# simonfuhrmann/mve

Measured on NVIDIA H100. Metric: mvs_depth_pixels_per_second, higher is better.
Workload: dtype f32

## Files before the change

### mve_b200/build.py

```python
from __future__ import annotations

import os
import subprocess

HERE = os.path.dirname(os.path.abspath(__file__))
ROOT = os.path.dirname(HERE)
LIB = os.path.join(HERE, "libb200mvs.so")
SOURCES = [os.path.join(HERE, "csrc", "b200mvs.cu"), os.path.join(HERE, "csrc", "depthmap.cu")]
DEPS = SOURCES + [os.path.join(HERE, "csrc", "patch_opt.cuh"), os.path.join(HERE, "csrc", "patch_thread.cuh"), os.path.join(HERE, "csrc", "patch_warp.cuh"),
               os.path.join(HERE, "csrc", "pset_device.cuh"), os.path.join(ROOT, "include", "b200mvs.h")]
NVCC_FLAGS = ["-gencode", "arch=compute_90a,code=sm_90a", "-lineinfo", "-O3", "-std=c++17",
              "-Xcompiler", "-fPIC", "-shared", "-Xptxas", "-v"]


def needs_build() -> bool:
    if not os.path.exists(LIB):
        return True
    t = os.path.getmtime(LIB)
    return any(os.path.getmtime(d) > t for d in DEPS)


def build(force: bool = False, verbose: bool = False) -> str:
    if not force and not needs_build():
        return LIB
    nvcc = os.environ.get("NVCC", "/usr/local/cuda/bin/nvcc")
    cmd = [nvcc] + NVCC_FLAGS + ["-o", LIB] + SOURCES
    res = subprocess.run(cmd, capture_output=True, text=True)
    if verbose or res.returncode != 0:
        print(res.stdout)
        print(res.stderr)
    if res.returncode != 0:
        raise RuntimeError("nvcc failed for libb200mvs.so")
    with open(os.path.join(HERE, "csrc", "ptxas_info.txt"), "w") as f:
        f.write(res.stderr)
    return LIB


if __name__ == "__main__":
    print(build(force=True, verbose=True))
```

### mve_b200/csrc/b200mvs.cu

```cuda
#include "../../include/b200mvs.h"
#include "patch_opt.cuh"
#include "patch_warp.cuh"
#include "patch_thread.cuh"
#include "pset_device.cuh"

#include <algorithm>
#include <cmath>
#include <cstdarg>
#include <cstddef>
#include <cstdio>
#include <cstring>
#include <cstdlib>
#include <functional>
#include <map>
#include <chrono>
#include <ctime>
#include <mutex>
#include <string>
#include <thread>
#include <atomic>
#include <vector>

using namespace b200mvs;

namespace {

thread_local std::string g_error;

struct HostLevel {
    int w = 0, h = 0, pitch = 0;
    float proj[9], invproj[9];
    uchar4* d_img = nullptr;
    uint4* d_quad = nullptr;
};

struct HostView {
    bool valid = false;
    bool has_image = false;
    int w = 0, h = 0;
    float flen = 0, paspect = 1, pp[2] = {0.5f, 0.5f}, rot[9], trans[3];
    float campos[3];
    float w2c[12];
    std::vector<HostLevel> lv;
    uchar4* d_base = nullptr;
    size_t bytes = 0;
    uint64_t last_use = 0;
};

size_t pyramid_bytes(const HostView& v)
{
    size_t texels = 0;
    for (const HostLevel& L : v.lv) texels += (size_t)L.pitch * L.h;
    return texels * (sizeof(uchar4) + sizeof(uint4));
}

// ... 545 lines not shown
    const int xs[4] = {max(0, x2 - 1), x2, min(iw - 1, x2 + 1), min(iw - 1, x2 + 2)};
    const float wr[4][4] = {{w3, w2, w2, w3}, {w2, w1, w1, w2}, {w2, w1, w1, w2}, {w3, w2, w2, w3}};
    float v0 = 0.f, v1 = 0.f, v2 = 0.f, ws = 0.f;
#pragma unroll
    for (int r = 0; r < 4; ++r) {
        const uchar4* row = in + (size_t)ys[r] * ipitch;
#pragma unroll
        for (int k = 0; k < 4; ++k) {
            const uchar4 t = row[xs[k]];
            v0 = __fadd_rn(v0, __fmul_rn((float)t.x, wr[r][k]));
            v1 = __fadd_rn(v1, __fmul_rn((float)t.y, wr[r][k]));
            v2 = __fadd_rn(v2, __fmul_rn((float)t.z, wr[r][k]));
            ws = __fadd_rn(ws, wr[r][k]);
        }
    }
    const float q0 = __fdiv_rn(v0, ws), q1 = __fdiv_rn(v1, ws), q2 = __fdiv_rn(v2, ws);
    uchar4 o;
    o.x = (unsigned char)(q0 > 0.f ? floorf(q0 + 0.5f) : ceilf(q0 - 0.5f));
    o.y = (unsigned char)(q1 > 0.f ? floorf(q1 + 0.5f) : ceilf(q1 - 0.5f));
    o.z = (unsigned char)(q2 > 0.f ? floorf(q2 + 0.5f) : ceilf(q2 - 0.5f));
    o.w = 255;
    out[(size_t)y * opitch + x] = o;
}

__global__ void k_make_quads(const uchar4* __restrict__ img, int w, int h, int pitch, uint4* __restrict__ quad)
{
    const int x = blockIdx.x * blockDim.x + threadIdx.x;
    const int y = blockIdx.y * blockDim.y + threadIdx.y;
    if (x >= w || y >= h) return;
    const int x1 = min(x + 1, w - 1), y1 = min(y + 1, h - 1);
    const unsigned* p = reinterpret_cast<const unsigned*>(img);
    uint4 q;
    q.x = p[(size_t)y * pitch + x]; q.y = p[(size_t)y * pitch + x1];
    q.z = p[(size_t)y1 * pitch + x]; q.w = p[(size_t)y1 * pitch + x1];
    quad[(size_t)y * pitch + x] = q;
}

__global__ void k_export_rgb(const uchar4* __restrict__ src, int w, int h, int pitch, uint8_t* __restrict__ dst)
{
    const int x = blockIdx.x * blockDim.x + threadIdx.x;
    const int y = blockIdx.y * blockDim.y + threadIdx.y;
    if (x >= w || y >= h) return;
    const uchar4 t = src[(size_t)y * pitch + x];
    uint8_t* p = dst + ((size_t)y * w + x) * 3;
    p[0] = t.x; p[1] = t.y; p[2] = t.z;
}

#ifndef OPT_MIN_BLOCKS
#define OPT_MIN_BLOCKS 1
#endif
constexpr int OPT_WARPS = OPT_TPB / 32;
using PatchT = b200mvs::PatchW;
using PatchT1 = b200mvs::PatchT;
constexpr size_t OPT_LUT_BYTES = sizeof(float) * (256 * LUT_STRIDE);
constexpr size_t OPT_SMEM_BYTES = OPT_LUT_BYTES + (size_t)OPT_TPB * sizeof(PatchT1) + PatchT1::MT_BYTES;
static_assert(OPT_SMEM_BYTES + 8 + 1024 <= 196 * 1024, "the patch kernels' shared memory must stay within the 196 KB carve-out");
__device__ __forceinline__ PatchT1& thread_patch(float* smem)
{
    return reinterpret_cast<PatchT1*>(reinterpret_cast<unsigned char*>(smem) + OPT_LUT_BYTES)[threadIdx.x];
}

__device__ __forceinline__ Entry load_entry(const Entry* p)
{
    const int4 a = __ldcg(reinterpret_cast<const int4*>(p));
    const int4 b = __ldcg(reinterpret_cast<const int4*>(p) + 1);
    Entry e;
    e.xy = a.x; e.jobdir = a.y; e.conf = __int_as_float(a.z); e.depth = __int_as_float(a.w);
    e.dzI = __int_as_float(b.x); e.dzJ = __int_as_float(b.y); e.slots = (unsigned)b.z; e.pad = b.w;
    return e;
}

__device__ __forceinline__ PatchIn patch_in(const Entry& e)
{
    PatchIn pi;
    pi.x = entry_x(e); pi.y = entry_y(e);
    pi.depth = e.depth; pi.dzI = e.dzI; pi.dzJ = e.dzJ; pi.slots = e.slots;
    return pi;
}

__device__ __forceinline__ unsigned long long global_timer_ns()
{
    unsigned long long t;
    asm volatile("mov.u64 %0, %%globaltimer;" : "=l"(t));
    return t;
}

__device__ __forceinline__ void optimise_entries(PatchT& p, const Entry* list, PatchOut* res, unsigned long long n,
                                                 unsigned long long* ticket, const JobParams* jobs, unsigned long long* counters)
{
    unsigned opts = 0u;
    for (;;) {
        unsigned long long w = 0ull;
        if (p.lane == 0) w = atomicAdd(ticket, 1ull);
        w = __shfl_sync(FULL, w, 0);
        if (w >= n) break;
        const Entry e = load_entry(&list[w]);
        p.begin(&jobs[entry_job(e)], patch_in(e));
        ++opts;
        while (!p.step()) {}
        PatchOut po;
        p.finish(po);
        if (p.lane == 0) res[w] = po;
    }
    if (p.lane == 0 && opts) {
        atomicAdd(&counters[C_SETS], (unsigned long long)p.n_sets);
        atomicAdd(&counters[C_OPTS], (unsigned long long)opts);
        p.n_sets = 0u;
    }
}

__device__ __forceinline__ void optimise_entries_t(PatchT1& p, const Entry* list, PatchOut* res, unsigned long long n,
                                                   unsigned long long* ticket, const JobParams* jobs, unsigned long long* counters)
{
    const int lane = threadIdx.x & 31;
    bool have = false;
    unsigned long long idx = 0ull;
    unsigned opts = 0u;
    for (;;) {
        if (!have) {
            const unsigned act = __activemask();
            const int leader = __ffs(act) - 1;
            unsigned long long base = 0ull;
            if (lane == leader) base = atomicAdd(ticket, (unsigned long long)__popc(act));
            base = __shfl_sync(act, base, leader);
            const unsigned long long w = base + (unsigned long long)__popc(act & ((1u << lane) - 1u));
            if (w >= n) break;
            idx = w;
            const Entry e = load_entry(&list[w]);
            p.begin(&jobs[entry_job(e)], patch_in(e));
            have = true;
            ++opts;
        }
        if (p.step()) {
            PatchOut po;
            p.finish(po);
            res[idx] = po;
            have = false;
        }
    }
    if (opts) {
        atomicAdd(&counters[C_SETS], (unsigned long long)p.n_sets);
        atomicAdd(&counters[C_OPTS], (unsigned long long)opts);
        p.n_sets = 0u;
    }
}

#ifndef OPT_THREAD_MIN
#define OPT_THREAD_MIN 8192
#endif

__global__ void __launch_bounds__(OPT_TPB, OPT_MIN_BLOCKS)
k_optimize(const Entry* __restrict__ in, PatchOut* __restrict__ out, int n, int mode,
           const DevSettings* __restrict__ st, const JobParams* __restrict__ jobs, const ViewParams* __restrict__ views,
           const float* __restrict__ g_lut, unsigned long long* counters)
{
    extern __shared__ float smem[];
    for (int i = threadIdx.x; i < 256 * LUT_STRIDE; i += blockDim.x) smem[i] = g_lut[i / LUT_STRIDE];
    __syncthreads();
    if (mode == 2 || (mode == 0 && n >= OPT_THREAD_MIN)) {
        PatchT1& p = thread_patch(smem);
        bind_thread(p, st, views, smem, (int)threadIdx.x);
        optimise_entries_t(p, in, out, (unsigned long long)n, &counters[C_TICKET], jobs, counters);
    } else {
        PatchT p;
        bind_thread(p, st, views, smem, (int)threadIdx.x);
        optimise_entries(p, in, out, (unsigned long long)n, &counters[C_TICKET], jobs, counters);
    }
}

__device__ __forceinline__ unsigned long long entry_key(const Entry& e)
{
    return ((unsigned long long)__float_as_uint(e.conf) << 8) | (unsigned long long)(7 - entry_dir(e));
}

struct FrontierParams {
    Entry* list[2];
    Entry* run;
    Entry* run2;
    unsigned* tile_cnt;
    unsigned long long* tile_off;
    long long n_tiles;
    PatchOut* res;
    unsigned char* written;
    unsigned long long cap;
    int n_seeds, n_jobs;
    const DevSettings* st;
    const JobParams* jobs;
    const ViewParams* views;
    const float* lut;
    unsigned long long* counters;
    FrontierCtl* ctl;
    unsigned* hist;
    int* thr_bin;
    HostMirror* host;
    volatile unsigned long long* host_filled;
    volatile int* host_cancel_job;
    int* job_cancel;
    long long thread_min;
    unsigned long long* job_run;
    int band_bins;
    int topk;
    int first_list;
};

__device__ __forceinline__ unsigned long long ld_relaxed_u64(const unsigned long long* p)
{
    unsigned long long v;
    asm volatile("ld.relaxed.gpu.global.u64 %0, [%1];" : "=l"(v) : "l"(p) : "memory");
    return v;
}
__device__ __forceinline__ void grid_barrier(unsigned long long* bar)
{
    __syncthreads();
    if (threadIdx.x == 0) {
        __threadfence();
// ... 217 lines not shown
        PHASE_END(PH_PICK);
        n_run = __ldcg(&ctl->nrun);
        if (lead) { ctl->nlist[p] = 0ull; ctl->need = 0ull; }
        }
        unsigned long long n_thread = 0ull;
        const Entry* run_cur = P.run;
        if (!seed_round && P.n_tiles > 0) {
            __shared__ unsigned long long s_big;
            if (threadIdx.x == 0) s_big = 0ull;
            __syncthreads();
            unsigned long long mine = 0ull;
            for (int j = threadIdx.x; j < P.n_jobs; j += blockDim.x) {
                const unsigned long long c = __ldcg(&P.job_run[j]);
                if (c >= (unsigned long long)P.thread_min) mine += c;
            }
            if (mine) atomicAdd(&s_big, mine);
            __syncthreads();
            n_thread = s_big;
        }
        if (n_thread > 0ull) {
            for (size_t i = gtid; i < n_run; i += gthreads) {
                const Entry e = load_entry(&P.run[i]);
                const int j = entry_job(e);
                if (__ldcg(&P.job_run[j]) < (unsigned long long)P.thread_min) continue;
                atomicAdd(&P.tile_cnt[tile_of(P.jobs[j], e)], 1u);
            }
            PHASE_END(PH_SORT);
            for (size_t b = gtid; b < (size_t)P.n_tiles; b += gthreads) {
                const unsigned c = __ldcg(&P.tile_cnt[b]);
                if (c) P.tile_off[b] = atomicAdd(&ctl->sort_cursor, (unsigned long long)c);
            }
            PHASE_END(PH_SORT);
            for (size_t i = gtid; i < n_run; i += gthreads) {
                const Entry e = load_entry(&P.run[i]);
                const int j = entry_job(e);
                if (__ldcg(&P.job_run[j]) < (unsigned long long)P.thread_min) {
                    P.run2[n_thread + take_slot(&ctl->small_cursor)] = e;
                    continue;
                }
                const long long bin = tile_of(P.jobs[j], e);
                const unsigned k = atomicSub(&P.tile_cnt[bin], 1u) - 1u;
                P.run2[__ldcg(&P.tile_off[bin]) + k] = e;
            }
            PHASE_END(PH_SORT);
            run_cur = P.run2;
        }
        const bool by_thread = n_thread > 0ull;
        if (by_thread) {
            PatchT1& pt = thread_patch(smem);
            bind_thread(pt, P.st, P.views, smem, (int)threadIdx.x);
            optimise_entries_t(pt, run_cur, P.res, n_thread, &ctl->ticket, P.jobs, cnt);
            __syncwarp();
        }
        if (n_run > n_thread) {
            PatchT pg;
            bind_thread(pg, P.st, P.views, smem, (int)threadIdx.x);
            optimise_entries(pg, run_cur + n_thread, P.res + n_thread, n_run - n_thread, by_thread ? &ctl->ticket2 : &ctl->ticket, P.jobs, cnt);
        }
        if (seed_round) {
            PHASE_END(PH_SEED);
            for (size_t i = gtid; i < (size_t)P.n_seeds; i += gthreads) {
                const float c = __ldcg(&P.res[i].conf);
                if (!(c > 0.f)) continue;
                atomicAdd(&cnt[C_SEED_OK], 1ull);
                const Entry e = load_entry(&run_cur[i]);
                const JobParams& J = P.jobs[entry_job(e)];
                atomicMax(&J.sel[pixel_of(J, e)], seed_key(c, i));
            }
            PHASE_END(PH_SELECT);
            for (size_t i = gtid; i < (size_t)P.n_seeds; i += gthreads) {
                const float c = __ldcg(&P.res[i].conf);
                if (!(c > 0.f)) continue;
                const Entry e = load_entry(&run_cur[i]);
                const int j = entry_job(e);
                const JobParams& J = P.jobs[j];
                const int idx = pixel_of(J, e);
                if (__ldcg(&J.sel[idx]) != seed_key(c, i)) continue;
                J.sel[idx] = 0ull;
                count_for_job(filled, j);
                const PatchOut r = load_result(&P.res[i]);
                write_pixel(J, idx, r);
                push_entry(P, 0, child_entry(e.xy, j, 4, r));
            }
            if (lead) ctl->ticket = 0ull;
            PHASE_END(PH_COMMIT);
            seed_round = false;
            p = 0;
            continue;
        }
        if (by_thread) PHASE_END(PH_OPT_THREAD); else PHASE_END(PH_OPT);
        for (size_t i = gtid; i < n_run; i += gthreads) {
            const Entry e = load_entry(&run_cur[i]);
            const PatchOut r = load_result(&P.res[i]);
            const int j = entry_job(e);
            const JobParams& J = P.jobs[j];
            const int idx = pixel_of(J, e);
            unsigned char w = 0;
            if (!(r.conf == 0.f)) {
                const float old = __ldcg(&J.conf[idx]);
                if (old <= 0.f) count_for_job(filled, j);
                if (old < r.conf) { write_pixel(J, idx, r); w = 1; }
            }
            P.written[i] = w;
            const unsigned act = __activemask(), wm = __ballot_sync(act, w);
            if (wm && lane == __ffs(act) - 1) atomicAdd(&ctl->need, 4ull * (unsigned long long)__popc(wm));
        }
        if (lead) {
// ... 436 lines not shown
{
    if (!ctx) return B200MVS_ERR_INVALID_ARG;
    std::lock_guard<std::mutex> lk(ctx->mtx);
    if (id < 0 || id >= (int)ctx->views.size() || !ctx->views[id].valid) return B200MVS_ERR_INVALID_ARG;
    return (int)ctx->views[id].lv.size();
}

int b200mvs_get_level(b200mvs_ctx* ctx, int id, int level, int* w, int* h, uint8_t* rgb)
{
    if (!ctx) return B200MVS_ERR_INVALID_ARG;
    std::lock_guard<std::mutex> lk(ctx->mtx);
    if (id < 0 || id >= (int)ctx->views.size() || !ctx->views[id].valid) return fail(B200MVS_ERR_INVALID_ARG, "invalid view");
    const HostView& v = ctx->views[id];
    if (level < 0 || level >= (int)v.lv.size()) return fail(B200MVS_ERR_INVALID_ARG, "invalid level");
    const HostLevel& L = v.lv[level];
    if (w) *w = L.w;
    if (h) *h = L.h;
    if (!rgb) return 0;
    if (ctx->device != B200MVS_DEVICE_NONE) CK(cudaSetDevice(ctx->device));
    pin_views(ctx, {id});
    int rc = load_views(ctx, {id}, nullptr);
    if (rc) return rc;
    uint8_t* d = nullptr;
    const size_t bytes = (size_t)L.w * L.h * 3;
    CK(dev_alloc(ctx, reinterpret_cast<void**>(&d), bytes));
    k_export_rgb<<<dim3((L.w + 31) / 32, (L.h + 7) / 8), dim3(32, 8), 0, ctx->stream>>>(L.d_img, L.w, L.h, L.pitch, d);
    cudaError_t e = cudaMemcpyAsync(rgb, d, bytes, cudaMemcpyDeviceToHost, ctx->stream);
    cudaStreamSynchronize(ctx->stream);
    dev_free(ctx, d, bytes);
    if (e != cudaSuccess) return fail(B200MVS_ERR_CUDA, "get_level copy: %s", cudaGetErrorString(e));
    return 0;
}

int b200mvs_global_view_selection(b200mvs_ctx* ctx, const b200mvs_settings* s, int ref, int32_t* ids_out, int cap)
{
    if (!ctx) return B200MVS_ERR_INVALID_ARG;
    std::lock_guard<std::mutex> lk(ctx->mtx);
    int rc;
    if ((rc = check_settings(s)) || (rc = check_ref_view(ctx, *s, ref))) return rc;
    if (cap > 0 && !ids_out) return fail(B200MVS_ERR_INVALID_ARG, "b200mvs_global_view_selection: ids_out is NULL");
    std::vector<int> sel;
    bool planned = false;
    {
        std::lock_guard<std::mutex> pl(ctx->plan_mtx);
        if (const HostPlan* p = find_plan(ctx, *s, ref)) { sel = p->gsel; planned = true; }
    }
    if (!planned) sel = global_view_selection(ctx, *s, ref);
    for (int i = 0; i < (int)sel.size() && i < cap; ++i) ids_out[i] = sel[i];
    return (int)sel.size();
}

int b200mvs_set_patch_mode(b200mvs_ctx* ctx, int mode, int64_t thread_min)
{
    if (!ctx || mode < 0 || mode > 2) return B200MVS_ERR_INVALID_ARG;
    std::lock_guard<std::mutex> lk(ctx->mtx);
    ctx->optimize_mode = mode;
    ctx->thread_min = thread_min;
    return 0;
}

int b200mvs_set_frontier_capacity(b200mvs_ctx* ctx, double entries_per_px, uint64_t min_entries)
{
    if (!ctx) return B200MVS_ERR_INVALID_ARG;
    std::lock_guard<std::mutex> lk(ctx->mtx);
    if (!std::isfinite(entries_per_px) || entries_per_px < 0.0 || entries_per_px > 64.0)
        return fail(B200MVS_ERR_INVALID_ARG, "frontier capacity: entries per pixel must be in [0, 64], got %g", entries_per_px);
    if (min_entries > (1ull << 40) || (entries_per_px == 0.0 && min_entries == 0))
        return fail(B200MVS_ERR_INVALID_ARG, "frontier capacity: min_entries must be at most 2^40, and at least 1 when entries per pixel is 0");
    ctx->frontier_cap.per_px = entries_per_px;
    ctx->frontier_cap.min = min_entries;
    return 0;
}

int b200mvs_frontier_info(b200mvs_ctx* ctx, uint64_t* initial_entries, uint64_t* final_entries, uint64_t* n_resumes)
{
    if (!ctx) return B200MVS_ERR_INVALID_ARG;
    std::lock_guard<std::mutex> lk(ctx->mtx);
    if (initial_entries) *initial_entries = ctx->fr_initial;
    if (final_entries) *final_entries = ctx->fr_final;
    if (n_resumes) *n_resumes = ctx->fr_resumes;
    return 0;
}

int b200mvs_plan_views(b200mvs_ctx* ctx, const b200mvs_settings* s, int n_refs, const int32_t* refs)
{
    if (!ctx) return B200MVS_ERR_INVALID_ARG;
    int rc = check_settings(s);
    if (rc) return rc;
    if (n_refs < 0 || (n_refs > 0 && !refs)) return fail(B200MVS_ERR_INVALID_ARG, "b200mvs_plan_views: bad arguments");
    std::vector<int> all(n_refs);
    for (int j = 0; j < n_refs; ++j) {
        if ((rc = check_ref_view(ctx, *s, refs[j]))) return rc;
        all[j] = j;
    }
    std::vector<HostPlan> made(n_refs);
    make_plans(ctx, *s, refs, all, made, nullptr);
    std::lock_guard<std::mutex> pl(ctx->plan_mtx);
    for (int j = 0; j < n_refs; ++j) ctx->plans[refs[j]] = std::move(made[j]);
    return 0;
}

int b200mvs_optimize_patches(b200mvs_ctx* ctx, const b200mvs_settings* s, int ref, const int32_t* gids, int ng,
                             const b200mvs_patch_in* in, int n, b200mvs_patch_out* out, b200mvs_stats* stats)
{
    if (!ctx) return B200MVS_ERR_INVALID_ARG;
    std::lock_guard<std::mutex> lk(ctx->mtx);
    int rc;
// ... 623 lines not shown
```

### mve_b200/csrc/patch_warp.cuh

```cuda
#pragma once
#include "patch_opt.cuh"

namespace b200mvs {

__device__ __forceinline__ float warp_sum(float v)
{
#pragma unroll
    for (int o = 16; o > 0; o >>= 1) v += __shfl_xor_sync(FULL, v, o);
    return v;
}
__device__ __forceinline__ double warp_sum(double v)
{
#pragma unroll
    for (int o = 16; o > 0; o >>= 1) v += __shfl_xor_sync(FULL, v, o);
    return v;
}
__device__ __forceinline__ float warp_max(float v)
{
#pragma unroll
    for (int o = 16; o > 0; o >>= 1) v = fmaxf(v, __shfl_xor_sync(FULL, v, o));
    return v;
}

__device__ __forceinline__ void warp_sum4(int lane, float& a, float& b, float& c, float& d)
// ... 133 lines not shown
            L.quad = reinterpret_cast<const uint4*>(__ldg(reinterpret_cast<const unsigned long long*>(&V->lv[l].quad)));
        }
        const bool aux = lane == NS;
        float qx, qy;
        project(w, L, aux ? cpx + crx : px, aux ? cpy + cry : py, aux ? cpz + crz : pz, qx, qy);
        const float ddx = __shfl_sync(FULL, qx, NS) - __shfl_sync(FULL, qx, CENTER);
        const float ddy = __shfl_sync(FULL, qy, NS) - __shfl_sync(FULL, qy, CENTER);
        const float dd2 = ddx * ddx + ddy * ddy;
        const float dd = dd2 * rsqrt_fast(dd2);
        const bool dok = dd > 0.f;
        const float step = rcp_fast(dd);
        const bool inb = qx > 0.f && qx < (float)(L.w - 1) && qy > 0.f && qy < (float)(L.h - 1);
        if (!__all_sync(FULL, inb || !act)) return 0u;
        if (act) {
            float gx = 0.f, gy = 0.f;
            if (dok) {
                float tx, ty;
                project(w, L, px + rx * step, py + ry * step, pz + rz * step, tx, ty);
                gx = tx - qx; gy = ty - qy;
            }
            const int left = (int)floorf(qx), top = (int)floorf(qy);
            const float fx = qx - (float)left, fy = qy - (float)top;
            const uint4 Q = __ldg(L.quad + (size_t)top * L.pitch + left);
            const float a[3] = {lut_k<0>(lut_tab, lane4, Q.x), lut_k<1>(lut_tab, lane4, Q.x), lut_k<2>(lut_tab, lane4, Q.x)};
            const float b[3] = {lut_k<0>(lut_tab, lane4, Q.y), lut_k<1>(lut_tab, lane4, Q.y), lut_k<2>(lut_tab, lane4, Q.y)};
            const float c[3] = {lut_k<0>(lut_tab, lane4, Q.z), lut_k<1>(lut_tab, lane4, Q.z), lut_k<2>(lut_tab, lane4, Q.z)};
            const float e[3] = {lut_k<0>(lut_tab, lane4, Q.w), lut_k<1>(lut_tab, lane4, Q.w), lut_k<2>(lut_tab, lane4, Q.w)};
#pragma unroll
            for (int ch = 0; ch < 3; ++ch) {
                const float x0 = (1.f - fx) * a[ch] + fx * b[ch];
                const float x3 = (1.f - fx) * c[ch] + fx * e[ch];
                n[ch] = (1.f - fy) * x0 + fy * x3;
                const float der = gx * (b[ch] - a[ch]) + gy * (c[ch] - a[ch]) + (gy * fx + gx * fy) * (a[ch] - b[ch] - c[ch] + e[ch]);
                d[ch] = dok ? der * dd : 0.f;
            }
        }
        return dok ? 3u : 1u;
    }

    __device__ __forceinline__ float ncc_of(const float (&n)[3]) const
    {
        const float inv_n = 1.f / (float)NS;
        float my0 = n[0], my1 = n[1], my2 = n[2], pad = 0.f;
        warp_sum4(lane, my0, my1, my2, pad);
        my0 *= inv_n; my1 *= inv_n; my2 *= inv_n;
        const float y0 = act ? n[0] - my0 : 0.f, y1 = act ? n[1] - my1 : 0.f, y2 = act ? n[2] - my2 : 0.f;
        float sqrDevY = y0 * y0 + y1 * y1 + y2 * y2;
        float devXY = e0 * y0 + e1 * y1 + e2 * y2;
        warp_sum2(lane, sqrDevY, devXY);
        const float p = sqrDevX * sqrDevY;
        return p > 0.f ? devXY * rsqrt_fast(p) : -1.f;
    }

    __device__ __forceinline__ void pass(bool candidates, bool cs_pending, bool want_ncc, bool want_normal, float*, PassOut& po)
    {
        float num = 0.f, den = 0.f;
        float A0 = 0.f, A1 = 0.f, A2 = 0.f, A3 = 0.f, A4 = 0.f, A5 = 0.f, B0 = 0.f, B1 = 0.f, B2 = 0.f;
        bool cs_active = cs_pending && st->use_color_scale;
        bool df_l = false;
        unsigned bits = 0u;
        const int count = candidates ? job->n_global : nsel();
        for (int k = 0; k < count; ++k) {
            int slot = k;
            if (candidates) { if (!((avail >> k) & 1u)) continue; }
            else slot = __shfl_sync(FULL, sel_l, k);
            float n[3], d[3];
            const unsigned r = sample(&views[job->gview[slot]], n, d);
            if (candidates) {
                const float v = (r & 1u) ? ncc_of(n) : -1.f;
                if (v < st->min_ncc) avail &= ~(1u << k);
                else if (lane == k) cand_ncc_l = v;
                continue;
            }
            if (r & 1u) bits |= 1u << (SH_COL + k);
            if (r & 2u) bits |= 1u << (SH_DER + k);
            if (want_ncc) {
                const float v = (r & 1u) ? ncc_of(n) : -1.f;
                if (lane == k) { df_l = fabsf(v - ncc_l) > st->min_refine_diff; ncc_l = v; }
            }
            float c0 = __shfl_sync(FULL, cs0_l, k), c1 = __shfl_sync(FULL, cs1_l, k), c2 = __shfl_sync(FULL, cs2_l, k);
            if (cs_active) {
                if (!(r & 1u)) cs_active = false;
                else {
                    float cc[3] = {c0, c1, c2};
                    float ab[3] = {(m0 - n[0] * c0) * n[0], (m1 - n[1] * c1) * n[1], (m2 - n[2] * c2) * n[2]};
                    float aa[3] = {n[0] * n[0], n[1] * n[1], n[2] * n[2]};
                    warp_sum4(lane, ab[0], ab[1], ab[2], aa[0]);
                    warp_sum2(lane, aa[1], aa[2]);
                    colour_scale_step(cc, ab, aa);
                    c0 = cc[0]; c1 = cc[1]; c2 = cc[2];
                    if (lane == k) { cs0_l = c0; cs1_l = c1; cs2_l = c2; }
                }
            }
            if ((r & 2u) && act) {
                const float g0 = c0 * d[0], g1 = c1 * d[1], g2 = c2 * d[2];
                const float r0 = m0 - c0 * n[0], r1 = m1 - c1 * n[1], r2 = m2 - c2 * n[2];
                num += g0 * r0 + g1 * r1 + g2 * r2;
                den += g0 * g0 + g1 * g1 + g2 * g2;
                if (want_normal) {
                    const float gg[3] = {g0, g1, g2};
                    const float rr[3] = {r0, r1, r2};
#pragma unroll
                    for (int ch = 0; ch < 3; ++ch) {
                        const float a0 = gg[ch];
                        const float a1 = fi * a0;
                        const float a2 = fj * a0;
                        A0 += a0 * a0; A1 += a0 * a1; A2 += a0 * a2;
                        A3 += a1 * a1; A4 += a1 * a2; A5 += a2 * a2;
                        B0 += a0 * rr[ch]; B1 += a1 * rr[ch]; B2 += a2 * rr[ch];
                    }
                }
            }
        }
        if (candidates) return;
        warp_sum2(lane, num, den);
        po.num = num; po.den = den;
        if (want_ncc) bits |= F_HAS_NCC | ((__ballot_sync(FULL, df_l) & 0xFu) << SH_DF);
        if (want_normal) bits |= F_HAS_NORMAL;
        pk = (pk & ~((0xFFu << SH_COL) | (want_ncc ? 0xFu << SH_DF : 0u) | F_HAS_NORMAL | F_HAS_NCC)) | bits;
        if (want_normal) {
            const double D0 = warp_sum((double)A0), D1 = warp_sum((double)A1), D2 = warp_sum((double)A2), D3 = warp_sum((double)A3);
            const double D4 = warp_sum((double)A4), D5 = warp_sum((double)A5);
            const double E0 = warp_sum((double)B0), E1 = warp_sum((double)B1), E2 = warp_sum((double)B2);
            const double m[9] = {D0, D1, D2, D1, D3, D4, D2, D4, D5};
            const double det = m[0] * m[4] * m[8] + m[1] * m[5] * m[6] + m[2] * m[3] * m[7]
                             - m[2] * m[4] * m[6] - m[1] * m[3] * m[8] - m[0] * m[5] * m[7];
            put(F_SINGULAR, det == 0.0);
            double inv[9];
            inv[0] = m[4] * m[8] - m[5] * m[7];
            inv[1] = m[2] * m[7] - m[1] * m[8];
            inv[2] = m[1] * m[5] - m[2] * m[4];
            inv[3] = m[5] * m[6] - m[3] * m[8];
            inv[4] = m[0] * m[8] - m[2] * m[6];
            inv[5] = m[2] * m[3] - m[0] * m[5];
            inv[6] = m[3] * m[7] - m[4] * m[6];
            inv[7] = m[1] * m[6] - m[0] * m[7];
            inv[8] = m[0] * m[4] - m[1] * m[3];
#pragma unroll
            for (int q = 0; q < 9; ++q) inv[q] /= det;
            po.nX0 = (float)(inv[0] * E0 + inv[1] * E1 + inv[2] * E2);
            po.nX1 = (float)(inv[3] * E0 + inv[4] * E1 + inv[5] * E2);
            po.nX2 = (float)(inv[6] * E0 + inv[7] * E1 + inv[8] * E2);
        }
    }

    __device__ __forceinline__ void sel_erase_mask(unsigned mask)
    {
        int src = 0, cnt = 0;
        for (int k = 0; k < MAX_LOCAL; ++k) {
            const bool kk = k < nsel() && !((mask >> k) & 1u);
            if (kk) { if (cnt == lane) src = k; ++cnt; }
        }
        const int s = __shfl_sync(FULL, sel_l, src);
        const float a = __shfl_sync(FULL, cs0_l, src), b = __shfl_sync(FULL, cs1_l, src), c = __shfl_sync(FULL, cs2_l, src);
        const float v = __shfl_sync(FULL, ncc_l, src);
        set_nsel(cnt);
        if (lane < cnt) { sel_l = s; cs0_l = a; cs1_l = b; cs2_l = c; ncc_l = v; }
        else { sel_l = 0xFF; }
    }
    __device__ __forceinline__ void sel_insert(int slot, float cs_init)
    {
        const int n = nsel();
        const unsigned smaller = __ballot_sync(FULL, lane < n && sel_l < slot);
        const int pos = __popc(smaller);
        const int s_up = __shfl_up_sync(FULL, sel_l, 1);
        const float a_up = __shfl_up_sync(FULL, cs0_l, 1), b_up = __shfl_up_sync(FULL, cs1_l, 1), c_up = __shfl_up_sync(FULL, cs2_l, 1);
        const float v_up = __shfl_up_sync(FULL, ncc_l, 1);
        if (lane > pos && lane <= n) { sel_l = s_up; cs0_l = a_up; cs1_l = b_up; cs2_l = c_up; ncc_l = v_up; }
        if (lane == pos) { sel_l = slot; cs0_l = cs1_l = cs2_l = cs_init; ncc_l = 0.f; }
        set_nsel(n + 1);
    }
    __device__ __forceinline__ unsigned low_ncc_mask() const
    {
        return __ballot_sync(FULL, lane < nsel() && ncc_l < st->accept_ncc);
    }

    __device__ __forceinline__ void lvs_greedy(const float*)
    {
        const unsigned N = st->nr_recon_neighbors;
        const float cs_init = 1.f / mm;
        float rdx = cpx - __ldg(&rv->campos[0]), rdy = cpy - __ldg(&rv->campos[1]), rdz = cpz - __ldg(&rv->campos[2]);
        {
            const float nn = sqrtf(rdx * rdx + rdy * rdy + rdz * rdz);
            rdx /= nn; rdy /= nn; rdz /= nn;
        }
        const int G = job->n_global;
        float vdx = 0.f, vdy = 0.f, vdz = 1.f, epx = 0.f, epy = 0.f, epz = 1.f, nfp = 1.f;
        if (lane < G) view_geometry(&views[job->gview[lane]], cpx, cpy, cpz, rdx, rdy, rdz, vdx, vdy, vdz, epx, epy, epz, nfp);
        bool found = true;
        while ((unsigned)nsel() < N && found) {
            found = false;
            const bool mine = lane < G && ((avail >> lane) & 1u);
            float score = -1.f;
            if (mine) {
                score = cand_ncc_l;
                if (mfp / nfp < 0.5f) score *= 0.01f;
// ... 83 lines not shown
```

Baseline: 70.72 million.

## Optimise small frontier runs with four-warp groups sharing one patch

Adds a PatchG variant in which a group of four warps cooperates on one patch optimisation. Each warp samples one selected or candidate view, and the warps exchange sample, NCC and colour-scale data through a per-group shared-memory buffer synchronised by an mbarrier. The frontier kernel switches to this grouped path by default when the run is small (no thread-per-patch work and fewer entries than the grid's groups), to raise parallelism in the tail where many warps would otherwise sit idle. In exchange it adds per-pass barrier synchronisation and shared-memory traffic, and it refactors the warp pass into gn_add, colour_scale_of and pass_end helpers.

```diff
diff --git a/mve_b200/build.py b/mve_b200/build.py
--- a/mve_b200/build.py
+++ b/mve_b200/build.py
@@ -7,7 +7,7 @@
 ROOT = os.path.dirname(HERE)
 LIB = os.path.join(HERE, "libb200mvs.so")
 SOURCES = [os.path.join(HERE, "csrc", "b200mvs.cu"), os.path.join(HERE, "csrc", "depthmap.cu")]
-DEPS = SOURCES + [os.path.join(HERE, "csrc", "patch_opt.cuh"), os.path.join(HERE, "csrc", "patch_thread.cuh"), os.path.join(HERE, "csrc", "patch_warp.cuh"),
+DEPS = SOURCES + [os.path.join(HERE, "csrc", "patch_opt.cuh"), os.path.join(HERE, "csrc", "patch_thread.cuh"), os.path.join(HERE, "csrc", "patch_warp.cuh"), os.path.join(HERE, "csrc", "patch_group.cuh"),
                os.path.join(HERE, "csrc", "pset_device.cuh"), os.path.join(ROOT, "include", "b200mvs.h")]
 NVCC_FLAGS = ["-gencode", "arch=compute_90a,code=sm_90a", "-lineinfo", "-O3", "-std=c++17",
               "-Xcompiler", "-fPIC", "-shared", "-Xptxas", "-v"]
diff --git a/mve_b200/csrc/b200mvs.cu b/mve_b200/csrc/b200mvs.cu
--- a/mve_b200/csrc/b200mvs.cu
+++ b/mve_b200/csrc/b200mvs.cu
@@ -1,6 +1,7 @@
 #include "../../include/b200mvs.h"
 #include "patch_opt.cuh"
 #include "patch_warp.cuh"
+#include "patch_group.cuh"
 #include "patch_thread.cuh"
 #include "pset_device.cuh"
 
@@ -652,12 +653,25 @@
 constexpr int OPT_WARPS = OPT_TPB / 32;
 using PatchT = b200mvs::PatchW;
 using PatchT1 = b200mvs::PatchT;
+using b200mvs::PatchG;
+#ifndef OPT_GROUPED
+#define OPT_GROUPED 1
+#endif
+constexpr int OPT_GROUPS = OPT_WARPS / b200mvs::GROUP_WARPS;
+static_assert(OPT_WARPS % b200mvs::GROUP_WARPS == 0, "whole groups of warps");
 constexpr size_t OPT_LUT_BYTES = sizeof(float) * (256 * LUT_STRIDE);
 constexpr size_t OPT_SMEM_BYTES = OPT_LUT_BYTES + (size_t)OPT_TPB * sizeof(PatchT1) + PatchT1::MT_BYTES;
 static_assert(OPT_SMEM_BYTES + 8 + 1024 <= 196 * 1024, "the patch kernels' shared memory must stay within the 196 KB carve-out");
 __device__ __forceinline__ PatchT1& thread_patch(float* smem)
 {
     return reinterpret_cast<PatchT1*>(reinterpret_cast<unsigned char*>(smem) + OPT_LUT_BYTES)[threadIdx.x];
+}
+
+static_assert((size_t)OPT_GROUPS * b200mvs::XB::GROUP_BYTES <= (size_t)OPT_TPB * sizeof(PatchT1) + PatchT1::MT_BYTES,
+              "the group exchange buffers must fit in the thread-per-patch part of the shared memory");
+__device__ __forceinline__ void bind_group(PatchG& p, const DevSettings* st, const ViewParams* views, float* smem)
+{
+    b200mvs::bind_group(p, st, views, smem, (int)threadIdx.x, reinterpret_cast<unsigned char*>(smem) + OPT_LUT_BYTES);
 }
 
 __device__ __forceinline__ Entry load_entry(const Entry* p)
@@ -707,6 +721,30 @@
         atomicAdd(&counters[C_OPTS], (unsigned long long)opts);
         p.n_sets = 0u;
     }
+}
+
+__device__ __forceinline__ void optimise_entries_g(PatchG& p, const Entry* list, PatchOut* res, unsigned long long n,
+                                                   unsigned long long* ticket, const JobParams* jobs, unsigned long long* counters)
+{
+    unsigned long long* const slots = reinterpret_cast<unsigned long long*>(p.xb);
+    const bool leader = p.gw == 0 && p.lane == 0;
+    unsigned opts = 0u;
+    for (unsigned it = 0u;; it ^= 1u) {
+        if (leader) slots[it] = atomicAdd(ticket, 1ull);
+        p.group_sync();
+        const unsigned long long w = slots[it];
+        if (w >= n) break;
+        const Entry e = load_entry(&list[w]);
+        p.begin(&jobs[entry_job(e)], patch_in(e));
+        ++opts;
+        while (!p.step()) {}
+        PatchOut po;
+        p.finish(po);
+        if (leader) res[w] = po;
+    }
+    if (p.lane == 0 && p.n_sets) atomicAdd(&counters[C_SETS], (unsigned long long)p.n_sets);
+    if (leader && opts) atomicAdd(&counters[C_OPTS], (unsigned long long)opts);
+    p.n_sets = 0u;
 }
 
 __device__ __forceinline__ void optimise_entries_t(PatchT1& p, const Entry* list, PatchOut* res, unsigned long long n,
@@ -761,6 +799,10 @@
         PatchT1& p = thread_patch(smem);
         bind_thread(p, st, views, smem, (int)threadIdx.x);
         optimise_entries_t(p, in, out, (unsigned long long)n, &counters[C_TICKET], jobs, counters);
+    } else if (mode == 3) {
+        PatchG p;
+        bind_group(p, st, views, smem);
+        optimise_entries_g(p, in, out, (unsigned long long)n, &counters[C_TICKET], jobs, counters);
     } else {
         PatchT p;
         bind_thread(p, st, views, smem, (int)threadIdx.x);
@@ -1084,7 +1126,11 @@
             optimise_entries_t(pt, run_cur, P.res, n_thread, &ctl->ticket, P.jobs, cnt);
             __syncwarp();
         }
-        if (n_run > n_thread) {
+        if (OPT_GROUPED && !by_thread && n_run <= (unsigned long long)gridDim.x * OPT_GROUPS) {
+            PatchG pg;
+            bind_group(pg, P.st, P.views, smem);
+            optimise_entries_g(pg, run_cur, P.res, n_run, &ctl->ticket, P.jobs, cnt);
+        } else if (n_run > n_thread) {
             PatchT pg;
             bind_thread(pg, P.st, P.views, smem, (int)threadIdx.x);
             optimise_entries(pg, run_cur + n_thread, P.res + n_thread, n_run - n_thread, by_thread ? &ctl->ticket2 : &ctl->ticket, P.jobs, cnt);
@@ -1627,7 +1673,7 @@
 
 int b200mvs_set_patch_mode(b200mvs_ctx* ctx, int mode, int64_t thread_min)
 {
-    if (!ctx || mode < 0 || mode > 2) return B200MVS_ERR_INVALID_ARG;
+    if (!ctx || mode < 0 || mode > 3) return B200MVS_ERR_INVALID_ARG;
     std::lock_guard<std::mutex> lk(ctx->mtx);
     ctx->optimize_mode = mode;
     ctx->thread_min = thread_min;
diff --git a/mve_b200/csrc/patch_group.cuh b/mve_b200/csrc/patch_group.cuh
--- /dev/null
+++ b/mve_b200/csrc/patch_group.cuh
@@ -0,0 +1,144 @@
+#pragma once
+#include "patch_warp.cuh"
+
+namespace b200mvs {
+
+constexpr int GROUP_WARPS = 4;
+constexpr int GROUP_THREADS = 32 * GROUP_WARPS;
+static_assert(MAX_LOCAL <= GROUP_WARPS, "a selected pass samples at most one view per warp");
+
+struct XB {
+    static constexpr int UNIFORM = 8;
+    static constexpr int VIEW = UNIFORM + 6 * 32;
+    static constexpr int CAND = MAX_LOCAL * VIEW;
+    static constexpr int PASS = CAND + MAX_GLOBAL;
+    static constexpr int TICKETS = 0;
+    static constexpr int BARRIER = 4;
+    static constexpr int HEAD = 8;
+    static constexpr int GROUP = HEAD + 2 * PASS;
+    static constexpr size_t GROUP_BYTES = sizeof(float) * GROUP;
+};
+static_assert(XB::GROUP % 4 == 0, "group exchange buffers stay 16-byte aligned");
+
+struct PatchG : PatchW {
+    float* xb;
+    int gw;
+    unsigned bar;
+    unsigned par;
+
+    __device__ __forceinline__ void group_sync() const
+    {
+        unsigned long long state;
+        asm volatile("mbarrier.arrive.shared::cta.b64 %0, [%1];" : "=l"(state) : "r"(bar) : "memory");
+        unsigned done;
+        do {
+            asm volatile("{\n\t.reg .pred p;\n\tmbarrier.try_wait.shared::cta.b64 p, [%1], %2;\n\tselp.u32 %0, 1, 0, p;\n\t}"
+                         : "=r"(done) : "r"(bar), "l"(state) : "memory");
+        } while (!done);
+    }
+
+    __device__ __forceinline__ void pass(bool candidates, bool cs_pending, bool want_ncc, bool want_normal, float*, PassOut& po)
+    {
+        float* const b = xb + XB::HEAD + par * XB::PASS;
+        par ^= 1u;
+        if (candidates) {
+            const int G = job->n_global;
+            for (int k = gw; k < G; k += GROUP_WARPS) {
+                if (!((avail >> k) & 1u)) continue;
+                float n[3], d[3];
+                const unsigned r = sample(&views[job->gview[k]], n, d);
+                const float v = (r & 1u) ? ncc_of(n) : -1.f;
+                if (lane == 0) b[XB::CAND + k] = v;
+            }
+            group_sync();
+            for (int k = 0; k < G; ++k) {
+                if (!((avail >> k) & 1u)) continue;
+                const float v = b[XB::CAND + k];
+                if (v < st->min_ncc) avail &= ~(1u << k);
+                else if (lane == k) cand_ncc_l = v;
+            }
+            return;
+        }
+        const int count = nsel();
+        const bool cs_on = cs_pending && st->use_color_scale;
+        float n[3], d[3];
+        unsigned r = 0u;
+        float* const u = b + gw * XB::VIEW;
+        if (gw < count) {
+            r = sample(&views[job->gview[__shfl_sync(FULL, sel_l, gw)]], n, d);
+            if (lane == 0) u[0] = __uint_as_float(r);
+#pragma unroll
+            for (int ch = 0; ch < 3; ++ch) {
+                u[XB::UNIFORM + ch * 32 + lane] = n[ch];
+                u[XB::UNIFORM + (3 + ch) * 32 + lane] = d[ch];
+            }
+        }
+        group_sync();
+        const bool exch = want_ncc || cs_on;
+        if (exch) {
+            if (gw < count) {
+                const float v = want_ncc ? ((r & 1u) ? ncc_of(n) : -1.f) : 0.f;
+                float c0 = __shfl_sync(FULL, cs0_l, gw), c1 = __shfl_sync(FULL, cs1_l, gw), c2 = __shfl_sync(FULL, cs2_l, gw);
+                bool active = cs_on && (r & 1u);
+                for (int j = 0; j < gw; ++j) active = active && (__float_as_uint(b[j * XB::VIEW]) & 1u);
+                bool fail = false;
+                if (active) {
+                    const unsigned pk0 = pk;
+                    pk |= F_OPTI;
+                    colour_scale_of(n, c0, c1, c2);
+                    fail = !is(F_OPTI);
+                    pk = pk0;
+                }
+                if (lane == 0) { u[1] = v; u[2] = c0; u[3] = c1; u[4] = c2; u[5] = fail ? 1.f : 0.f; }
+            }
+            group_sync();
+        }
+        GNSums s = {0.f, 0.f, 0.f, 0.f, 0.f, 0.f, 0.f, 0.f, 0.f, 0.f, 0.f};
+        bool cs_active = cs_on;
+        bool df_l = false;
+        unsigned bits = 0u;
+        for (int k = 0; k < count; ++k) {
+            const float* const w = b + k * XB::VIEW;
+            const unsigned rk = __float_as_uint(w[0]);
+            if (rk & 1u) bits |= 1u << (SH_COL + k);
+            if (rk & 2u) bits |= 1u << (SH_DER + k);
+            if (want_ncc) {
+                const float v = w[1];
+                if (lane == k) { df_l = fabsf(v - ncc_l) > st->min_refine_diff; ncc_l = v; }
+            }
+            float c0, c1, c2;
+            if (exch) { c0 = w[2]; c1 = w[3]; c2 = w[4]; }
+            else { c0 = __shfl_sync(FULL, cs0_l, k); c1 = __shfl_sync(FULL, cs1_l, k); c2 = __shfl_sync(FULL, cs2_l, k); }
+            if (cs_active) {
+                if (!(rk & 1u)) cs_active = false;
+                else {
+                    if (w[5] != 0.f) pk &= ~F_OPTI;
+                    if (lane == k) { cs0_l = c0; cs1_l = c1; cs2_l = c2; }
+                }
+            }
+            if ((rk & 2u) && act) {
+                const float nk[3] = {w[XB::UNIFORM + lane], w[XB::UNIFORM + 32 + lane], w[XB::UNIFORM + 64 + lane]};
+                const float dk[3] = {w[XB::UNIFORM + 96 + lane], w[XB::UNIFORM + 128 + lane], w[XB::UNIFORM + 160 + lane]};
+                gn_add(s, rk, c0, c1, c2, nk, dk, want_normal);
+            }
+        }
+        pass_end(s, bits, df_l, want_ncc, want_normal, po);
+    }
+
+    __device__ __forceinline__ bool step() { return auto_step(*this); }
+};
+
+__device__ __forceinline__ void bind_group(PatchG& p, const DevSettings* st, const ViewParams* views, const float* lut_rep, int tid,
+                                           unsigned char* smem)
+{
+    bind_thread(p, st, views, lut_rep, tid);
+    const int g = tid / GROUP_THREADS;
+    p.gw = (tid / 32) % GROUP_WARPS;
+    p.xb = reinterpret_cast<float*>(smem + (size_t)g * XB::GROUP_BYTES);
+    p.bar = (unsigned)__cvta_generic_to_shared(p.xb + XB::BARRIER);
+    p.par = 0u;
+    if (tid % GROUP_THREADS == 0) asm volatile("mbarrier.init.shared::cta.b64 [%0], %1;" :: "r"(p.bar), "r"(GROUP_THREADS) : "memory");
+    __syncthreads();
+}
+
+}
diff --git a/mve_b200/csrc/patch_warp.cuh b/mve_b200/csrc/patch_warp.cuh
--- a/mve_b200/csrc/patch_warp.cuh
+++ b/mve_b200/csrc/patch_warp.cuh
@@ -209,10 +209,79 @@
         return p > 0.f ? devXY * rsqrt_fast(p) : -1.f;
     }
 
+    struct GNSums { float num, den, A0, A1, A2, A3, A4, A5, B0, B1, B2; };
+
+    __device__ __forceinline__ void gn_add(GNSums& s, unsigned r, float c0, float c1, float c2, const float (&n)[3],
+                                           const float (&d)[3], bool want_normal) const
+    {
+        if ((r & 2u) && act) {
+            const float g0 = c0 * d[0], g1 = c1 * d[1], g2 = c2 * d[2];
+            const float r0 = m0 - c0 * n[0], r1 = m1 - c1 * n[1], r2 = m2 - c2 * n[2];
+            s.num += g0 * r0 + g1 * r1 + g2 * r2;
+            s.den += g0 * g0 + g1 * g1 + g2 * g2;
+            if (want_normal) {
+                const float gg[3] = {g0, g1, g2};
+                const float rr[3] = {r0, r1, r2};
+#pragma unroll
+                for (int ch = 0; ch < 3; ++ch) {
+                    const float a0 = gg[ch];
+                    const float a1 = fi * a0;
+                    const float a2 = fj * a0;
+                    s.A0 += a0 * a0; s.A1 += a0 * a1; s.A2 += a0 * a2;
+                    s.A3 += a1 * a1; s.A4 += a1 * a2; s.A5 += a2 * a2;
+                    s.B0 += a0 * rr[ch]; s.B1 += a1 * rr[ch]; s.B2 += a2 * rr[ch];
+                }
+            }
+        }
+    }
+
+    __device__ __forceinline__ void colour_scale_of(const float (&n)[3], float& c0, float& c1, float& c2)
+    {
+        float cc[3] = {c0, c1, c2};
+        float ab[3] = {(m0 - n[0] * c0) * n[0], (m1 - n[1] * c1) * n[1], (m2 - n[2] * c2) * n[2]};
+        float aa[3] = {n[0] * n[0], n[1] * n[1], n[2] * n[2]};
+        warp_sum4(lane, ab[0], ab[1], ab[2], aa[0]);
+        warp_sum2(lane, aa[1], aa[2]);
+        colour_scale_step(cc, ab, aa);
+        c0 = cc[0]; c1 = cc[1]; c2 = cc[2];
+    }
+
+    __device__ __forceinline__ void pass_end(GNSums& s, unsigned bits, bool df_l, bool want_ncc, bool want_normal, PassOut& po)
+    {
+        warp_sum2(lane, s.num, s.den);
+        po.num = s.num; po.den = s.den;
+        if (want_ncc) bits |= F_HAS_NCC | ((__ballot_sync(FULL, df_l) & 0xFu) << SH_DF);
+        if (want_normal) bits |= F_HAS_NORMAL;
+        pk = (pk & ~((0xFFu << SH_COL) | (want_ncc ? 0xFu << SH_DF : 0u) | F_HAS_NORMAL | F_HAS_NCC)) | bits;
+        if (want_normal) {
+            const double D0 = warp_sum((double)s.A0), D1 = warp_sum((double)s.A1), D2 = warp_sum((double)s.A2), D3 = warp_sum((double)s.A3);
+            const double D4 = warp_sum((double)s.A4), D5 = warp_sum((double)s.A5);
+            const double E0 = warp_sum((double)s.B0), E1 = warp_sum((double)s.B1), E2 = warp_sum((double)s.B2);
+            const double m[9] = {D0, D1, D2, D1, D3, D4, D2, D4, D5};
+            const double det = m[0] * m[4] * m[8] + m[1] * m[5] * m[6] + m[2] * m[3] * m[7]
+                             - m[2] * m[4] * m[6] - m[1] * m[3] * m[8] - m[0] * m[5] * m[7];
+            put(F_SINGULAR, det == 0.0);
+            double inv[9];
+            inv[0] = m[4] * m[8] - m[5] * m[7];
+            inv[1] = m[2] * m[7] - m[1] * m[8];
+            inv[2] = m[1] * m[5] - m[2] * m[4];
+            inv[3] = m[5] * m[6] - m[3] * m[8];
+            inv[4] = m[0] * m[8] - m[2] * m[6];
+            inv[5] = m[2] * m[3] - m[0] * m[5];
+            inv[6] = m[3] * m[7] - m[4] * m[6];
+            inv[7] = m[1] * m[6] - m[0] * m[7];
+            inv[8] = m[0] * m[4] - m[1] * m[3];
+#pragma unroll
+            for (int q = 0; q < 9; ++q) inv[q] /= det;
+            po.nX0 = (float)(inv[0] * E0 + inv[1] * E1 + inv[2] * E2);
+            po.nX1 = (float)(inv[3] * E0 + inv[4] * E1 + inv[5] * E2);
+            po.nX2 = (float)(inv[6] * E0 + inv[7] * E1 + inv[8] * E2);
+        }
+    }
+
     __device__ __forceinline__ void pass(bool candidates, bool cs_pending, bool want_ncc, bool want_normal, float*, PassOut& po)
     {
-        float num = 0.f, den = 0.f;
-        float A0 = 0.f, A1 = 0.f, A2 = 0.f, A3 = 0.f, A4 = 0.f, A5 = 0.f, B0 = 0.f, B1 = 0.f, B2 = 0.f;
+        GNSums s = {0.f, 0.f, 0.f, 0.f, 0.f, 0.f, 0.f, 0.f, 0.f, 0.f, 0.f};
         bool cs_active = cs_pending && st->use_color_scale;
         bool df_l = false;
         unsigned bits = 0u;
@@ -239,66 +308,14 @@
             if (cs_active) {
                 if (!(r & 1u)) cs_active = false;
                 else {
-                    float cc[3] = {c0, c1, c2};
-                    float ab[3] = {(m0 - n[0] * c0) * n[0], (m1 - n[1] * c1) * n[1], (m2 - n[2] * c2) * n[2]};
-                    float aa[3] = {n[0] * n[0], n[1] * n[1], n[2] * n[2]};
-                    warp_sum4(lane, ab[0], ab[1], ab[2], aa[0]);
-                    warp_sum2(lane, aa[1], aa[2]);
-                    colour_scale_step(cc, ab, aa);
-                    c0 = cc[0]; c1 = cc[1]; c2 = cc[2];
+                    colour_scale_of(n, c0, c1, c2);
                     if (lane == k) { cs0_l = c0; cs1_l = c1; cs2_l = c2; }
                 }
             }
-            if ((r & 2u) && act) {
-                const float g0 = c0 * d[0], g1 = c1 * d[1], g2 = c2 * d[2];
-                const float r0 = m0 - c0 * n[0], r1 = m1 - c1 * n[1], r2 = m2 - c2 * n[2];
-                num += g0 * r0 + g1 * r1 + g2 * r2;
-                den += g0 * g0 + g1 * g1 + g2 * g2;
-                if (want_normal) {
-                    const float gg[3] = {g0, g1, g2};
-                    const float rr[3] = {r0, r1, r2};
-#pragma unroll
-                    for (int ch = 0; ch < 3; ++ch) {
-                        const float a0 = gg[ch];
-                        const float a1 = fi * a0;
-                        const float a2 = fj * a0;
-                        A0 += a0 * a0; A1 += a0 * a1; A2 += a0 * a2;
-                        A3 += a1 * a1; A4 += a1 * a2; A5 += a2 * a2;
-                        B0 += a0 * rr[ch]; B1 += a1 * rr[ch]; B2 += a2 * rr[ch];
-                    }
-                }
-            }
+            gn_add(s, r, c0, c1, c2, n, d, want_normal);
         }
         if (candidates) return;
-        warp_sum2(lane, num, den);
-        po.num = num; po.den = den;
-        if (want_ncc) bits |= F_HAS_NCC | ((__ballot_sync(FULL, df_l) & 0xFu) << SH_DF);
-        if (want_normal) bits |= F_HAS_NORMAL;
-        pk = (pk & ~((0xFFu << SH_COL) | (want_ncc ? 0xFu << SH_DF : 0u) | F_HAS_NORMAL | F_HAS_NCC)) | bits;
-        if (want_normal) {
-            const double D0 = warp_sum((double)A0), D1 = warp_sum((double)A1), D2 = warp_sum((double)A2), D3 = warp_sum((double)A3);
-            const double D4 = warp_sum((double)A4), D5 = warp_sum((double)A5);
-            const double E0 = warp_sum((double)B0), E1 = warp_sum((double)B1), E2 = warp_sum((double)B2);
-            const double m[9] = {D0, D1, D2, D1, D3, D4, D2, D4, D5};
-            const double det = m[0] * m[4] * m[8] + m[1] * m[5] * m[6] + m[2] * m[3] * m[7]
-                             - m[2] * m[4] * m[6] - m[1] * m[3] * m[8] - m[0] * m[5] * m[7];
-            put(F_SINGULAR, det == 0.0);
-            double inv[9];
-            inv[0] = m[4] * m[8] - m[5] * m[7];
-            inv[1] = m[2] * m[7] - m[1] * m[8];
-            inv[2] = m[1] * m[5] - m[2] * m[4];
-            inv[3] = m[5] * m[6] - m[3] * m[8];
-            inv[4] = m[0] * m[8] - m[2] * m[6];
-            inv[5] = m[2] * m[3] - m[0] * m[5];
-            inv[6] = m[3] * m[7] - m[4] * m[6];
-            inv[7] = m[1] * m[6] - m[0] * m[7];
-            inv[8] = m[0] * m[4] - m[1] * m[3];
-#pragma unroll
-            for (int q = 0; q < 9; ++q) inv[q] /= det;
-            po.nX0 = (float)(inv[0] * E0 + inv[1] * E1 + inv[2] * E2);
-            po.nX1 = (float)(inv[3] * E0 + inv[4] * E1 + inv[5] * E2);
-            po.nX2 = (float)(inv[6] * E0 + inv[7] * E1 + inv[8] * E2);
-        }
+        pass_end(s, bits, df_l, want_ncc, want_normal, po);
     }
 
     __device__ __forceinline__ void sel_erase_mask(unsigned mask)
```

Result: no change. 71.22 million, median of 6 (+0.7%).
